# kubernetes-sigs/kube-batch

Hardware: AMD Instinct MI355X
Metric: pod-node scoring evals/sec + binds/sec, 100k tasks x 10k nodes snapshot (higher is better)
Workload: dtype f64+i64

## Files before the change

kube-batch_amd/csrc/kb_commit_sel.hip:

```cpp
#include <string.h>

#include <algorithm>

#include "kb_k9.hpp"
#include "kb_repair.hpp"

#define K9S_PREP0 5u
#define K9S_PREPS 3u
#define K9S_SPIN_LIMIT (1u << 21)

__device__ __forceinline__ uint32_t k9s_ld(const uint32_t *p) { return __hip_atomic_load(p, __ATOMIC_ACQUIRE, __HIP_MEMORY_SCOPE_WORKGROUP); }
__device__ __forceinline__ void k9s_st(uint32_t *p, uint32_t v) { __hip_atomic_store(p, v, __ATOMIC_RELEASE, __HIP_MEMORY_SCOPE_WORKGROUP); }
__device__ __forceinline__ bool k9s_wait(K9Sync &Y, const uint32_t *p, uint32_t need, uint32_t nap = 1u) {
  uint32_t spins = 0;
  for (;;) {
    if (k9s_ld(p) >= need) return true;
    if ((++spins & 31u) == 0u) {
      if (k9s_ld(&Y.stop) | k9s_ld(&Y.err)) return k9s_ld(p) >= need;
      if (spins > K9S_SPIN_LIMIT) { k9s_st(&Y.err, 1u); return false; }
    }
    if (nap == 0u) { } else if (nap == 1u) __builtin_amdgcn_s_sleep(1); else if (nap <= 4u) __builtin_amdgcn_s_sleep(4); else __builtin_amdgcn_s_sleep(16);
  }
}

__global__ void __launch_bounds__(K9_THREADS) k_commit_select(const K9KernArgs ka) {
  KbCommitArgs a = ka.hot;
  {
    const unsigned char __attribute__((address_space(4))) *kp = (const unsigned char __attribute__((address_space(4))) *)__builtin_amdgcn_kernarg_segment_ptr();
    a.dev = (const KbDev *)(kp + offsetof(K9KernArgs, dev));
    a.round = (const KbRound *)(kp + offsetof(K9KernArgs, round));
  }
  extern __shared__ __align__(16) unsigned char k9_smem[];
  if ((blockIdx.x & 7u) != 0u && a.round->lists_ready != nullptr) {
    const uint32_t row = blockIdx.x - 1u - blockIdx.x / 8u;
    if (row < a.n_mrows && !KB_CHAIN_BROKEN(*a.round)) kb_repair_row<K9_THREADS>(*a.dev, *a.round, k9_smem, row, threadIdx.x);
    return;
  }
  if (k9_preamble(a)) return;
  const uint32_t tid = threadIdx.x, lane = tid & 63, wave = tid >> 6;
  const uint32_t S = a.n_mrows, W = a.n_rows;
  const K9Layout lo = k9_layout(W, S, a.L, a.NP, a.R, true);
  unsigned char *k9_base_ = k9_smem;
  K9_LDS_VIEWS(lo)
  (void)shp; (void)S; (void)dk; (void)ckey; (void)cpos;
  K9Sel &X = *reinterpret_cast<K9Sel *>(k9_smem + lo.sel);
  K9Sync &Y = X.sync;
  const unsigned long long t_start = wall_clock64();
#ifdef KB_K9_TRACE
  unsigned long long t_stage[2] = {0ull, 0ull};
  const bool staged = k9_prologue(a, lo, k9_smem, tid, 0u, t_stage);
#else
  const bool staged = k9_prologue(a, lo, k9_smem, tid, 0u);
#endif
  if (!staged) {
    if (tid == 0) k9_publish_skipped(a);
    return;
  }

  uint32_t job_of_my_row = 0u;
  if (tid < W) job_of_my_row = a.dev->t_job[desc[tid].task];
  if (tid < 8) { X.brk[tid] = 0u; X.stm[tid] = 0u; }
  if (tid < 4) { X.stat[tid] = 0u; X.tr[tid] = 0u; }
  if (tid < sizeof(K9Sync) / 4) reinterpret_cast<uint32_t *>(&Y)[tid] = 0u;
  __syncthreads();
  if (tid < W) {
    bool brk = tid == 0;
    if (tid) {
      const KbRowDesc &p = desc[tid - 1], &q = desc[tid];
      const bool plain = (p.flags & 1u) && (p.resmask == 0u || (p.flags & 4u));
      brk = !(plain && !(p.flags & 2u) && q.slot == p.slot && q.flags == p.flags && q.resmask == p.resmask);
    }
    if (brk) atomicOr(&X.brk[tid >> 5], 1u << (tid & 31));
  }
  __syncthreads();
  if (tid < W) {
    uint32_t w = tid >> 5, mword = X.brk[w] & (0xFFFFFFFFu >> (31u - (tid & 31u)));
    while (mword == 0u) { w--; mword = X.brk[w]; }
    const uint32_t p = 32u * w + (31u - (uint32_t)__clz((int)mword));
    if ((tid - p) % K9_SEL_MAXRUN == 0u) atomicOr(&X.stm[tid >> 5], 1u << (tid & 31));
  }
  __syncthreads();
  if (tid < W && ((X.stm[tid >> 5] >> (tid & 31)) & 1u)) {
    uint32_t kidx = (uint32_t)__popc(X.stm[tid >> 5] & ((1u << (tid & 31)) - 1u));
    for (uint32_t w = 0; w < (tid >> 5); w++) kidx += (uint32_t)__popc(X.stm[w]);
    X.runs[kidx] = (uint16_t)tid;
  }
  __syncthreads();
  uint32_t K = 0;
  for (uint32_t w = 0; w < 8; w++) K += (uint32_t)__popc(X.stm[w]);
  {
    uint4 rr = make_uint4(0u, 0u, 0u, 0u);
    uint32_t i0c = 0u;
    uint32_t rlen = 0u;
    if (tid < K) { i0c = X.runs[tid]; rr = rinfo[i0c]; rlen = ((tid + 1u < K) ? (uint32_t)X.runs[tid + 1u] : W) - i0c; }
    __syncthreads();
    if (tid < K) rinfo[tid] = make_uint4(i0c | (rlen << 16), rr.y, rr.z, rr.w);
    __syncthreads();
  }

#ifdef KB_K9_TRACE
  uint32_t tacc[10] = {0, 0, 0, 0, 0, 0, 0, 0, 0, 0};
  const unsigned long long t_tab = wall_clock64();
  tacc[1] = (uint32_t)(t_stage[0] - t_start); tacc[9] = (uint32_t)(t_stage[1] - t_stage[0]); tacc[2] = (uint32_t)(t_tab - t_stage[1]);
  unsigned long long tlast = __builtin_readcyclecounter();
#define K9S_TR(k, t0) do { if (lane == 0) atomicAdd(&X.tr[k], (uint32_t)(__builtin_readcyclecounter() - (t0))); } while (0)
#define K9S_NOW() __builtin_readcyclecounter()
#else
#define K9S_TR(k, t0) do { (void)(t0); } while (0)
#define K9S_NOW() 0ull
#endif
#ifndef KB_K9_NAP_PREP
#define KB_K9_NAP_PREP 1u
#endif
  constexpr uint32_t nap_prep = KB_K9_NAP_PREP, nap_dk = 1u;
#if !defined(KB_K9_PRIO) || KB_K9_PRIO
#define K9S_SETPRIO(p) __builtin_amdgcn_s_setprio(p)
#else
#define K9S_SETPRIO(p) do { } while (0)
#endif
  const unsigned long long lt = (1ull << lane) - 1ull;
  gptrd gi, gr;
  { const KbDev &d = *a.dev; gi = (gptrd)d.idle; gr = (gptrd)d.rel; }
#define K9S_RUN_HEADER_OF(ri_)                                                                                         \
  const uint32_t hx_ = (uint32_t)__builtin_amdgcn_readfirstlane((int)(ri_).x);                                          \
  const uint32_t i0 = hx_ & 0xFFFFu, r = hx_ >> 16, s = (uint32_t)__builtin_amdgcn_readfirstlane((int)(ri_).y);          \
  const uint32_t fl0 = (uint32_t)__builtin_amdgcn_readfirstlane((int)(ri_).z), km0 = (uint32_t)__builtin_amdgcn_readfirstlane((int)(ri_).w); \
  const bool plain0 = (fl0 & 1u) && (km0 == 0u || (fl0 & 4u));                                                         \
  const bool sel_run = !a.backfill && plain0 && r >= 2u && a.whole;             \
  (void)sel_run; (void)i0;
#define K9S_RUN_SHAPE(kk)                                                                                              \
  const K9Shape sh = shapes[s];                                                                                        \
  const double *si = sinit + (size_t)s * RS;                                                                           \
  const double *rres = rowres + ((kk) % K9S_PREPS) * (uint32_t)a.R;    \
  const double *rqv = plain0 ? si : rres + 2;                                             \
  (void)rqv; (void)rres;
#define K9S_RUN_HEADER(kk)                                                                                             \
  const uint4 ri_ = rinfo[(kk)];                                                                                       \
  K9S_RUN_HEADER_OF(ri_)                                                                                               \
  K9S_RUN_SHAPE(kk)

  if (wave == 0) {
    K9S_SETPRIO(3);
    uint32_t nd = 0, n_dirty_rows = 0, n_runs = 0, n_slow = 0, i_end = 0, reason_end = KB_REASON_DONE;
    uint32_t prev_nd0 = 0, prev_pc = 0;
    bool prev_chg = true;
    bool prev_all = false;
    uint4 hd_next = rinfo[0];
    for (uint32_t k = 0; k < K; k++) {
      uint32_t lane_i = tid;
      asm volatile("" : "+v"(lane_i));
      const uint4 hd = hd_next;
      if (k + 1u < K) hd_next = rinfo[k + 1u];
      K9S_RUN_HEADER_OF(hd)
      K9_STAMP(3);
      {
        uint32_t spins = 0;
        bool ok = true;
        for (;;) {
          const uint32_t *wp = (lane_i == 0u) ? (prev_all ? &Y.seq_spec : &Y.seq_cand) : (prev_chg ? &Y.seq_dk[(lane_i - 1u) & 3u] : &Y.seq_early[(lane_i - 1u) & 3u]);
          const uint32_t v = (lane_i < 5u) ? k9s_ld(wp) : 0xFFFFFFFFu;
          if (__ballot(v < k + 1u) == 0ull) break;
          if ((++spins & 31u) == 0u && (k9s_ld(&Y.err) || spins > K9S_SPIN_LIMIT)) { k9s_st(&Y.err, 1u); ok = false; break; }
          __builtin_amdgcn_s_sleep(1);
        }
        if (!ok) { reason_end = KB_REASON_INTERNAL; i_end = i0; break; }
      }
      if (prev_all && lane_i == 0) k9s_st(&Y.seq_cand, k + 1u);
// ... 320 lines not shown
          else if (lane_i == F_PORTS) cur8 |= sh.want;
          else if (lane_i == F_CLS_LEFT) cur8 -= (1ull << 32);
          uint32_t bulk = 1u;
          if (bf_bulk) {
            const uint32_t left1 = (uint32_t)(rl64(cur8, F_CLS_LEFT) >> 32);
            bulk = 1u + min(r - j - 1u, left1);
            if (bulk > 1u) {
              if (lane_i == F_NZC) { double z = u2d(cur8); for (uint32_t t = 1; t < bulk; t++) z += sh.nzc; cur8 = d2u(z); }
              else if (lane_i == F_NZM) { double z = u2d(cur8); for (uint32_t t = 1; t < bulk; t++) z += sh.nzm; cur8 = d2u(z); }
              else if (lane_i == F_CLS_LEFT) cur8 -= ((unsigned long long)(bulk - 1u) << 32);
            }
          }
          if (lane_i < K9_NF) st[lane_i] = cur8;
          if (lane_i < bulk) ldec[i0 + j + lane_i] = (unsigned long long)n | ((unsigned long long)kind << 32);
          j += bulk - 1u;
          n_dirty += bulk - 1u;
          K9_WAVE_FENCE();
          const bool more = j + 1u < r && !kind;
          const uint32_t adjm1 = (!kind && has_map) ? km0 : 0u;
          uint32_t nk = 0u;
          if (more) nk = k9_eval_v(a, sh, k9_load(st), scs, gi, gr, si, adjm1, 1.0, rqv, nb, nmaskbits);
          if (km0 && has_map) {
            if (sc_lane && ((km0 >> sd) & 1u)) k9_sc_sub(kind ? gr : gi, a.NP, sd, n, rqv[sd]);
            sc_dirty = 1;
          }
          if (more) {
            if (lane_i == L) {
              if (is_new) k1 = nk;
              else if (wsel == 0) d0 = nk; else if (wsel == 1) d1 = nk; else if (wsel == 2) d2 = nk; else d3 = nk;
            }
            m = wave_max_u32(max(max(max(d0, d1), max(d2, d3)), (lane_i < pc) ? k1 : 0u));
          }
          n_dirty++;
        }
        if (kind) { j++; reason = KB_REASON_PIPELINED; break; }
      }
      }
      if (sc_dirty) __threadfence();
      const uint32_t i_next = i0 + j;
      uint32_t stop = (reason != KB_REASON_DONE || k + 1u >= K) ? 1u : 0u;
      if (!stop && a.has_aff && !a.backfill && i_next != 0u) {
        const uint32_t fln = (uint32_t)__builtin_amdgcn_readfirstlane((int)hd_next.z);
        if (fln & 2u) { reason = KB_REASON_RENORM; stop = 1u; }
      }
      if (pc) { const uint32_t cp = rl32(cpos, pc - 1u); if (lane_i == 0) cursor[s] = cp + 1u; }
      prev_nd0 = nd; prev_pc = pc; prev_all = pc == ncand;
      K9_WAVE_FENCE();
      prev_chg = chg_any;
      nd += pc; n_dirty_rows += n_dirty; n_runs += 1u; n_slow += plain0 ? 0u : 1u;
      i_end = i_next; reason_end = reason;
      if (lane_i == 0) {
        Y.nd_at[(k + 1u) & 3u] = nd;
        Y.spec_ok[(k + 1u) & 3u] = prev_all ? 1u : 0u;
        if (stop) k9s_st(&Y.stop, 1u);
        k9s_st(&Y.seq_done, k + 1u);
      }
      if (stop) break;
    }
#ifdef KB_K9_TRACE
    tacc[4] = (uint32_t)(wall_clock64() - t_tab);
#endif
    if (lane == 0) {
      if (k9s_ld(&Y.err)) reason_end = KB_REASON_INTERNAL;
      k9s_st(&Y.stop, 1u);
      H.i = i_end; H.nd = nd; H.reason = reason_end; H.n_dirty_rows = n_dirty_rows; H.n_runs = n_runs; H.n_slow = n_slow;
    }
  } else if (wave <= 4u) {
    K9S_SETPRIO(2);
    const uint32_t t = tid - 64u;
    for (uint32_t q = 0; q < K; q++) {
      K9S_RUN_HEADER(q)
      uint32_t *dko = X.dkb[q & 1u];
      uint32_t key = 0u, nd_early = 0u;
      const unsigned long long tw0 = K9S_NOW();
      if (q >= 1u) {
        if (!k9s_wait(Y, &Y.seq_done, q - 1u, nap_dk) || !k9s_wait(Y, &Y.seq_cand, q, nap_dk) || k9s_ld(&Y.stop)) break;
        nd_early = Y.nd_at[(q - 1u) & 3u] + Y.ncand_at[(q - 1u) & 3u];
        if (t < nd_early) {
          const K9St vs = k9_load(slots + (size_t)t * K9_NF);
          const K9Sc scp = k9_sc_preload(sh.active >> 2, gi, gr, a.NP, vs.node);
          key = k9_eval_v(a, sh, vs, scp, gi, gr, si, 0u, 0.0, si, nb, nmaskbits);
          dko[t] = key;
        }
        const uint32_t wmo = wave_max_u32(t < Y.nd_at[(q - 1u) & 3u] ? key : 0u);
        if (lane == 0) Y.mdko[q & 1u][wave - 1u] = wmo;
      }
      if (lane == 0) k9s_st(&Y.seq_early[wave - 1u], q + 1u);
      if (wave == 1u) K9S_TR(3, tw0);
      const unsigned long long tw1 = K9S_NOW();
      if (!k9s_wait(Y, &Y.seq_done, q, nap_dk) || k9s_ld(&Y.stop)) break;
      if (wave == 1u) K9S_TR(2, tw1);
      const uint32_t nd = Y.nd_at[q & 3u];
      if (t < nd && (t >= nd_early || ((Y.chg[(q - 1u) & 1u][t >> 5] >> (t & 31)) & 1u))) {
        const K9St vs = k9_load(slots + (size_t)t * K9_NF);
        const K9Sc scp = k9_sc_preload(sh.active >> 2, gi, gr, a.NP, vs.node);
        key = k9_eval_v(a, sh, vs, scp, gi, gr, si, 0u, 0.0, si, nb, nmaskbits);
      }
      if (t >= nd) key = 0u;
      if (t < K9_MAXSLOTS) dko[t] = key;
      const uint32_t wm = wave_max_u32(key);
      if (lane == 0) { Y.mdk[q & 1u][wave - 1u] = wm; k9s_st(&Y.seq_dk[wave - 1u], q + 1u); }
    }
  } else if (wave < K9S_PREP0 + K9S_PREPS) {
    typedef const unsigned long long __attribute__((address_space(1))) *gptr8;
    typedef const uint32_t __attribute__((address_space(1))) *gptr4;
    gptr8 g8[10];
    gptr8 gports;
    gptr4 gcls, gmaxp, gpodc, gnm;
    {
      const KbDev &d = *a.dev;
      g8[0] = (gptr8)reinterpret_cast<const unsigned long long *>(d.idle); g8[1] = (gptr8)reinterpret_cast<const unsigned long long *>(d.idle + d.NP);
      g8[2] = (gptr8)reinterpret_cast<const unsigned long long *>(d.rel); g8[3] = (gptr8)reinterpret_cast<const unsigned long long *>(d.rel + d.NP);
      g8[4] = (gptr8)reinterpret_cast<const unsigned long long *>(d.inv_acpu); g8[5] = (gptr8)reinterpret_cast<const unsigned long long *>(d.inv_amem);
      g8[6] = (gptr8)reinterpret_cast<const unsigned long long *>(d.acpu); g8[7] = (gptr8)reinterpret_cast<const unsigned long long *>(d.amem);
      g8[8] = (gptr8)reinterpret_cast<const unsigned long long *>(d.nzc); g8[9] = (gptr8)reinterpret_cast<const unsigned long long *>(d.nzm);
      gports = (gptr8)d.ports;
      gcls = (gptr4)d.ncls; gmaxp = (gptr4)reinterpret_cast<const uint32_t *>(d.maxpods); gpodc = (gptr4)reinterpret_cast<const uint32_t *>(d.podcnt); gnm = (gptr4)d.nmask;
    }
    K9Prep &P = X.prep[wave - K9S_PREP0];
    for (uint32_t m = wave - K9S_PREP0; m < K; m += K9S_PREPS) {
      K9S_RUN_HEADER(m)
      const uint32_t r1 = m >= 1u ? (uint32_t)X.runs[m] - (uint32_t)X.runs[m - 1u] : 0u, r2 = m >= 2u ? (uint32_t)X.runs[m - 1u] - (uint32_t)X.runs[m - 2u] : 0u;
      uint32_t want = r + r1 + r2, need = m >= 2u ? m - 2u : 0u;
      if (want > 64u) { want = r + r1; need = m >= 1u ? m - 1u : 0u; }
      const unsigned long long tp0 = K9S_NOW();
      if (!k9s_wait(Y, &Y.seq_done, need, nap_prep) || k9s_ld(&Y.stop)) break;
      K9S_TR(1, tp0);
      uint32_t nf = 0;
      {
        uint32_t e_ = cursor[s];
        while (nf < want) {
          const uint32_t pos_ = e_ + lane;
          const uint32_t kk_ = (pos_ < Lp) ? lists[s * Lp + pos_] : 0u;
          const bool nz_ = kk_ != 0u;
          const uint32_t nn_ = nmaskbits - (kk_ & nmaskbits);
          const bool cl_ = nz_ && !((bitmap[(nz_ ? nn_ : 0u) >> 5] >> (nn_ & 31)) & 1u);
          const unsigned long long zeros_ = __ballot(!nz_);
          const uint32_t fz_ = zeros_ ? (uint32_t)__ffsll((unsigned long long)zeros_) - 1u : 64u;
          const unsigned long long clean_ = __ballot(cl_ && lane < fz_);
          const uint32_t rank_ = (uint32_t)__popcll(clean_ & lt);
          if (((clean_ >> lane) & 1ull) && nf + rank_ < want) { P.ckey[nf + rank_] = kk_; P.cpos[nf + rank_] = pos_; }
          nf = min(want, nf + (uint32_t)__popcll(clean_));
          if (fz_ < 64u || e_ + 64u >= Lp) break;
          e_ += 64u;
        }
        K9_WAVE_FENCE();
      }
      const uint32_t key = (lane < nf) ? P.ckey[lane] : 0u, mypos = (lane < nf) ? P.cpos[lane] : 0u;
      const uint32_t n = nmaskbits - (key & nmaskbits);
      unsigned long long raw[11] = {0, 0, 0, 0, 0, 0, 0, 0, 0, 0, 0};
      uint32_t rcls = 0, rmaxp = 0, rpodc = 0, rnm = 0;
      if (lane < nf) {
#pragma unroll
        for (int f = 0; f < 10; f++) raw[f] = g8[f][n];
        raw[F_PORTS] = gports ? gports[n] : 0ull;
// ... 109 lines not shown
```

kube-batch_amd/csrc/kb_engine.cpp:

```cpp
#include "kb_engine_int.hpp"

thread_local std::string g_create_err;

namespace kbe {

void ensure_window_buffers(kb_engine *e, uint32_t rows) {
  if (rows <= e->win_cap) return;
  if (!e->b_desc.p) e->b_desc.alloc(sizeof(KbRowDesc) * 2 * KB_K5_MAX_WINDOW);
  e->h_rows.resize(rows);
  e->h_slot.resize(rows);
  e->h_decnode.resize(rows);
  e->h_deckind.resize(rows);
  e->win_cap = rows;
}
void ensure_ip_scratch(kb_engine *e, size_t rows) {
  if (!e->hs.has_interpod) return;
  const size_t NP = e->dev.NP;
  if (e->b_ip_scnt.bytes < sizeof(long long) * rows * NP) {
    e->b_ip_scnt.alloc(sizeof(long long) * rows * NP);
    e->b_ip_shist.alloc(sizeof(int32_t) * rows * NP);
  }
  e->dev.ip_scratch_cnt = e->b_ip_scnt.as<long long>();
  e->dev.ip_scratch_hist = e->b_ip_shist.as<int32_t>();
}
// ... 130 lines not shown
        else if (ck[0] == 's') eng->commit_pin = KB_COMMIT_SELECT;
        if (eng->commit_pin >= 0) eng->commit_kernel = eng->commit_pin;
      }
      eng->fast_rounds = !(eng->flags & KB_FLAG_SYNC_ROUNDS);
      const char *cr = getenv("KB_CHAIN_ROUNDS");
      eng->chain_rounds = !(cr && cr[0] == '0');
      const char *pb = getenv("KB_PROBE");
      eng->probe_enabled = !(pb && pb[0] == '0');
      const char *ov = getenv("KB_OVERLAP");
      eng->overlap = !(ov && ov[0] == '0');
      const char *fr = getenv("KB_FUSE_REPAIR");
      eng->fuse_repair = !(fr && fr[0] == '0');
      const char *wf = getenv("KB_DEVICE_WATERFILL");
      eng->device_waterfill = !(wf && wf[0] == '0');
    }
    e = eng.release();
  });
  if (rc == KB_OK) *out = e;
  return rc;
}

void kb_engine_destroy(kb_engine *e) {
  if (!e) return;
  if (getenv("KB_K5_STATS"))
    fprintf(stderr, "[kb K5] rounds on the run kernel %llu, on the selection kernel %llu, last dirty share %.3f\n",
            (unsigned long long)e->rounds_run, (unsigned long long)e->rounds_sel, e->dirty_share);
  if (getenv("KB_K5_STATS") && e->rounds_sel)
    fprintf(stderr, "[kb select] runs of >= 2 rows: all picks clean first placements %llu, committed by shots %llu (shots cut short by a table's end %llu; shots %llu)\n",
            (unsigned long long)e->sel_stat[0], (unsigned long long)e->sel_stat[1], (unsigned long long)e->sel_stat[2], (unsigned long long)e->sel_stat[3]);
  if (getenv("KB_K5_STATS"))
    fprintf(stderr, "[kb K5] rounds %llu, rows %llu, dirty slots %llu, dirty-won rows %llu, runs %llu, runs with a row-specific Resreq %llu (%llu)\n",
            (unsigned long long)e->stats.rounds, (unsigned long long)e->stats.decisions, (unsigned long long)e->k5_slots,
            (unsigned long long)e->stats.row_fallbacks, (unsigned long long)e->k5_walks, (unsigned long long)e->k5_rescans,
            (unsigned long long)e->k5_demand);
  if (getenv("KB_K5_STATS")) fprintf(stderr, "[kb overlap] rounds with candidate lists built beside the predecessor's commit %llu, lists that never arrived %llu; repair launches: %.3f ms from their start to the tag seen\n",
                                     (unsigned long long)e->overlapped_rounds, (unsigned long long)e->overlap_faults, e->tl_repair_tag);
  if (getenv("KB_K5_STATS"))
    fprintf(stderr, "[kb host] ms over the engine's life: reset %.2f, allocate up to its first launch %.2f, speculation breaks (answer -> re-planned launch) %.2f, "
            "closing reductions %.2f, waiting for rounds %.2f, backfill up to its first launch %.2f\n", e->tl_reset, e->tl_begin, e->tl_break, e->tl_finish, e->tl_wait, e->tl_backfill);
  if (getenv("KB_K5_STATS"))
    fprintf(stderr, "[kb host] of the start: order machine %.2f, first probe %.2f, first plan %.2f; of the breaks: probe launch + absorb %.2f, waiting for the probe %.2f, re-plan %.2f\n",
            e->tl_begin_parts[0], e->tl_begin_parts[1], e->tl_begin_parts[2], e->tl_break_parts[0], e->tl_break_parts[1], e->tl_break_parts[2]);
  if (getenv("KB_K5_STATS")) fprintf(stderr, "[kb probe] %llu probes, %llu shapes marked dead by them\n", (unsigned long long)e->probes, (unsigned long long)e->probe_deaths);
  if (getenv("KB_K5_STATS") && e->k5_trace[0] > 0) {
    static const char *ph[10] = {"barrier 1 (wave 0's wait)", "evaluate: candidates (wave 0)", "barrier 2", "rows", "prepare the next run",
                                "rows, of runs with scalar dimensions", "runs with scalar dimensions (count)", "evaluate, of runs with scalar dimensions",
                                "dirty-winner entries (count)", "loop top"};
    static const char *ph_sel[10] = {"wave 0 waits for candidates + dirty keys", "staging: lists, descriptors (10 ns units, not clocks)", "run tables (10 ns units)", "rows: serial loop, tail, publish", "wave 0's loop (10 ns units)",
                                    "selection: entries + first rank", "selection: deep passes", "selection: picks + AddTask", "selection: all picks clean", "shape tables (10 ns units)"};
    const double runs = (double)(e->k5_walks ? e->k5_walks : 1);
    for (int k = 0; k < 10; k++) fprintf(stderr, "[kb K5 trace] %-32s %14.0f clocks  (%.0f per run)\n", e->rounds_sel > e->rounds_run ? ph_sel[k] : ph[k], e->k5_trace[k], e->k5_trace[k] / runs);
    static const char *ph_role[4] = {"prep waves wait for their run's turn (sum of 3)", "prep waves wait for the walk's turn (sum of 3)", "wave 1 waits for the previous run", "wave 1 evaluates + publishes"};
    if (e->rounds_sel > e->rounds_run) for (int k = 10; k < 14; k++) fprintf(stderr, "[kb K5 trace] %-32s %14.0f clocks  (%.0f per run)\n", ph_role[k - 10], e->k5_trace[k], e->k5_trace[k] / runs);
  }
  (void)hipSetDevice(e->device);
  delete e;
}

int kb_get_binds(kb_engine *e, uint32_t *task_node_out) {
  if (!e) return KB_E_INVALID;
  return guarded(e, [&]() {
    if (!e->loaded) throw EngineError(KB_E_STATE, "no session loaded");
    quiesce(e);
    HIP_OK(hipMemcpy(task_node_out, e->b_tbind.p, sizeof(uint32_t) * e->hs.T, hipMemcpyDeviceToHost));
    uint64_t nb = 0;
    for (uint32_t t = 0; t < e->hs.T; t++) nb += task_node_out[t] != KB_NONE;
    e->stats.binds = nb;
  });
}

int kb_get_task_state(kb_engine *e, uint8_t *status_out, uint32_t *node_out) {
  if (!e) return KB_E_INVALID;
  return guarded(e, [&]() {
    if (!e->loaded) throw EngineError(KB_E_STATE, "no session loaded");
    quiesce(e);
    if (status_out) HIP_OK(hipMemcpy(status_out, e->b_tstatus.p, e->hs.T, hipMemcpyDeviceToHost));
    if (node_out) HIP_OK(hipMemcpy(node_out, e->b_tnode.p, sizeof(uint32_t) * e->hs.T, hipMemcpyDeviceToHost));
  });
}

int kb_get_node_state(kb_engine *e, double *idle, double *releasing, int64_t *nz_cpu, int64_t *nz_mem, int32_t *pod_cnt) {
  if (!e) return KB_E_INVALID;
  return guarded(e, [&]() {
    if (!e->loaded) throw EngineError(KB_E_STATE, "no session loaded");
    quiesce(e);
    const uint32_t N = e->hs.N, NP = e->dev.NP;
    const int R = e->hs.R;
    if (idle) HIP_OK(hipMemcpy2D(idle, sizeof(double) * N, e->b_idle.p, sizeof(double) * NP, sizeof(double) * N, R, hipMemcpyDeviceToHost));
    if (releasing) HIP_OK(hipMemcpy2D(releasing, sizeof(double) * N, e->b_rel.p, sizeof(double) * NP, sizeof(double) * N, R, hipMemcpyDeviceToHost));
    if (nz_cpu) HIP_OK(hipMemcpy(nz_cpu, e->b_nzc.p, sizeof(int64_t) * N, hipMemcpyDeviceToHost));
    if (nz_mem) HIP_OK(hipMemcpy(nz_mem, e->b_nzm.p, sizeof(int64_t) * N, hipMemcpyDeviceToHost));
    if (pod_cnt) HIP_OK(hipMemcpy(pod_cnt, e->b_podcnt.p, sizeof(int32_t) * N, hipMemcpyDeviceToHost));
  });
}

int kb_get_shares(kb_engine *e, double *job_share, double *queue_share, double *queue_deserved) {
  if (!e) return KB_E_INVALID;
  return guarded(e, [&]() {
    if (!e->loaded) throw EngineError(KB_E_STATE, "no session loaded");
    const HostSession &hs = e->hs;
    if (job_share) std::memcpy(job_share, hs.job_share.data(), sizeof(double) * hs.J);
    if (queue_share) std::memcpy(queue_share, hs.queue_share.data(), sizeof(double) * hs.Q);
    if (queue_deserved)
      for (uint32_t q = 0; q < hs.Q; q++)
        for (int d = 0; d < hs.R; d++) queue_deserved[(size_t)d * hs.Q + q] = hs.deserved[q].get(d);
  });
// ... 25 lines not shown
```

kube-batch_amd/csrc/kb_k9.hpp:

```cpp
#pragma once
#include <hip/hip_runtime.h>
#include <stddef.h>
#include <stdint.h>
#include <stdlib.h>

#include "kb_device.h"
#include "kb_eval.hpp"
#include "kb_warm.hpp"

#define K9_THREADS 512
#define K9_MAXRUN 64
#define K9_SEL_MAXRUN 32
#define K9_MAXSLOTS 256
#define K9_NF 13
enum { F_IDLE0 = 0, F_IDLE1, F_REL0, F_REL1, F_INVAC, F_INVAM, F_AC, F_AM, F_NZC, F_NZM, F_PORTS, F_CLS_LEFT, F_NODE_NMASK };

struct K9Shape {
  double init0, init1, nzc, nzm;
  unsigned long long conf, want;
  uint32_t cls, active, crow, pad;
};

struct K9Hdr {
  uint32_t i, nd, reason, stop;
  uint32_t ncand, n_dirty_rows, n_runs, n_slow;
  uint32_t cur_s, cur_r, cur_fl, cur_km;
};

struct K9Prep {
  uint32_t ckey[64], cpos[64];
};
struct K9Sync {
  uint32_t seq_done;
  uint32_t seq_cand;
  uint32_t seq_dk[4];
  uint32_t seq_early[4];
  uint32_t seq_spec;
  uint32_t spec_ok[4];
  uint32_t stop, err;
  uint32_t nd_at[4];
  uint32_t ncand_at[4];
  uint32_t mdk[2][4];
  uint32_t mdko[2][4];
  uint32_t chg[2][10];
};
struct K9Sel {
  K9Sync sync;
  K9Prep prep[3];
  uint16_t runs[KB_K5_MAX_ROWS];
  uint32_t brk[8], stm[8];
  struct Cand { uint32_t ckey[64], cpos[64], ckind[64], ck1[64], crnm[64]; } cand[2];
  uint32_t dkb[2][K9_MAXSLOTS];
  uint32_t c_slot[64], c_sorted[64];
  alignas(16) uint32_t c_key[64];
  alignas(16) uint32_t e_eff[64];
  uint32_t e_key[64];
  uint32_t pool[K9_MAXSLOTS + 64];
  uint32_t tr[4];
  uint32_t stat[4];
};

struct K9Layout {
  uint32_t slots, rowres, sinit, shapes, desc, rinfo, dec, hdr, dk, ckey, cpos, cursor, shp, lists, bitmap, sel, total;
  uint32_t Lp, RS;
};
__host__ __device__ inline K9Layout k9_layout(uint32_t n_rows, uint32_t n_shapes, uint32_t L, uint32_t NP, int R, bool sel = false) {
  K9Layout o;
  o.RS = R > 2 ? (uint32_t)(R - 2) : 0u;
  o.Lp = L;
  uint32_t off = 0;
  o.slots = off;  off += (n_rows + K9_MAXRUN) * K9_NF * 8u;
  o.rowres = off; off += 3u * (uint32_t)R * 8u;
  o.sinit = off;  off += n_shapes * o.RS * 8u;
  o.shapes = off; off += n_shapes * (uint32_t)sizeof(K9Shape);
  o.desc = off;   off += n_rows * (uint32_t)sizeof(KbRowDesc);
  off = (off + 15u) & ~15u;
  o.rinfo = off;  off += n_rows * 16u;
  o.dec = off;    off += n_rows * 8u;
  o.hdr = off;    off += (uint32_t)sizeof(K9Hdr);
  o.dk = off;     off += K9_MAXSLOTS * 4u;
  o.ckey = off;   off += K9_MAXRUN * 4u;
  o.cpos = off;   off += K9_MAXRUN * 4u;
  o.cursor = off; off += n_shapes * 4u;
  o.shp = off;    off += n_shapes * 4u;
  o.lists = off;  off += n_shapes * o.Lp * 4u;
  o.bitmap = off; off += (NP / 32u) * 4u;
  off = (off + 15u) & ~15u;
  o.sel = 0;
  if (sel) { o.sel = off; off += (uint32_t)sizeof(K9Sel); }
  o.total = (off + 15u) & ~15u;
  return o;
}

__device__ __forceinline__ uint32_t wave_max_u32(uint32_t v) {
#define K9_UMAX(ctrl, row_mask) v = max(v, (uint32_t)__builtin_amdgcn_update_dpp((int)v, (int)v, (ctrl), (row_mask), 0xf, false))
  K9_UMAX(0xB1, 0xf);
  K9_UMAX(0x4E, 0xf);
// ... 135 lines not shown
  if (a.round->chain_expect != 0u && *a.round->chain != a.round->chain_expect) {
    if (threadIdx.x == 0 && blockIdx.x == 0) k9_publish_skipped(a);
    return true;
  }
  if (blockIdx.x != 0) {
    if ((blockIdx.x & 7u) != 0u) return true;
    const uint32_t h = blockIdx.x / 8u - 1u, lines = a.NP / 16;
    if (h >= KB_WARM_HELPERS) return true;
    const uint32_t l0 = (uint32_t)(((unsigned long long)h * lines) / KB_WARM_HELPERS), l1 = (uint32_t)(((unsigned long long)(h + 1) * lines) / KB_WARM_HELPERS);
    const unsigned long long acc = kb_warm_lines(*a.dev, a.keys, 0, l0, l1, threadIdx.x, K9_THREADS);
    if (acc == 0x123456789abcdefull) a.result[15] = 1;
    return true;
  }
  return false;
}

#define K9_LDS_VIEWS(lo)                                                                                           \
  unsigned long long *slots = reinterpret_cast<unsigned long long *>(k9_base_ + lo.slots); \
  double *rowres = reinterpret_cast<double *>(k9_base_ + lo.rowres); \
  double *sinit = reinterpret_cast<double *>(k9_base_ + lo.sinit); \
  K9Shape *shapes = reinterpret_cast<K9Shape *>(k9_base_ + lo.shapes); \
  KbRowDesc *desc = reinterpret_cast<KbRowDesc *>(k9_base_ + lo.desc); \
  uint4 *rinfo = reinterpret_cast<uint4 *>(k9_base_ + lo.rinfo); \
  unsigned long long *ldec = reinterpret_cast<unsigned long long *>(k9_base_ + lo.dec); \
  K9Hdr &H = *reinterpret_cast<K9Hdr *>(k9_base_ + lo.hdr); \
  uint32_t *dk = reinterpret_cast<uint32_t *>(k9_base_ + lo.dk); \
  uint32_t *ckey = reinterpret_cast<uint32_t *>(k9_base_ + lo.ckey); \
  uint32_t *cpos = reinterpret_cast<uint32_t *>(k9_base_ + lo.cpos); \
  uint32_t *cursor = reinterpret_cast<uint32_t *>(k9_base_ + lo.cursor); \
  uint32_t *shp = reinterpret_cast<uint32_t *>(k9_base_ + lo.shp); \
  uint32_t *lists = reinterpret_cast<uint32_t *>(k9_base_ + lo.lists); \
  uint32_t *bitmap = reinterpret_cast<uint32_t *>(k9_base_ + lo.bitmap); \
  const uint32_t RS = lo.RS, Lp = lo.Lp; \
  const uint32_t nb = a.node_bits, nmaskbits = (1u << nb) - 1u;

template <bool ACQ>
__device__ __forceinline__ bool k9_wait_tags(const KbCommitArgs &a, K9Hdr &H, const uint32_t *tags, const uint32_t tag, const uint32_t n, const uint32_t tid) {
  if (tid < n) {
    bool gone = false;
    uint32_t spins = 0;
    while ((ACQ ? __hip_atomic_load(&tags[tid], __ATOMIC_ACQUIRE, __HIP_MEMORY_SCOPE_AGENT) : __hip_atomic_load(&tags[tid], __ATOMIC_RELAXED, __HIP_MEMORY_SCOPE_AGENT)) != tag) {
      __builtin_amdgcn_s_sleep(2);
      if ((++spins & 15u) == 0u) {
        if (a.round->chain_expect != 0u && __hip_atomic_load(a.round->chain, __ATOMIC_RELAXED, __HIP_MEMORY_SCOPE_AGENT) != a.round->chain_expect) { gone = true; break; }
        if (spins > (1u << 22)) { gone = true; break; }
      }
    }
    if (gone) H.stop = 1u;
  }
  __syncthreads();
  return H.stop == 0u;
}

__device__ __forceinline__ bool k9_prologue(const KbCommitArgs &a, const K9Layout &lo, unsigned char *k9_base_, const uint32_t tid, const uint32_t maxrun,
                                            unsigned long long *stamps = nullptr) {
  const uint32_t S = a.n_mrows, W = a.n_rows;
  K9_LDS_VIEWS(lo)
  (void)slots; (void)rowres; (void)ldec; (void)dk; (void)ckey; (void)cpos; (void)RS;
  const bool fused = a.round->lists_ready != nullptr;
  for (uint32_t w = tid; w < a.NP / 32; w += K9_THREADS) bitmap[w] = 0;
  if (tid == 0) { H.i = 0; H.nd = 0; H.reason = KB_REASON_DONE; H.stop = 0; H.ncand = 0; H.n_dirty_rows = 0; H.n_runs = 0; H.n_slow = 0; H.cur_s = 0; H.cur_r = 0; H.cur_fl = 0; H.cur_km = 0; }
  if (fused) {
    __syncthreads();
    if (!k9_wait_tags<true>(a, H, a.round->ready, a.round->ready_tag, S, tid)) return false;
  }
  constexpr uint32_t UD = 4, UL = 16;
  const uint32_t tot = S * Lp;
  auto stage_lists = [&](uint32_t lbase0) {
    for (uint32_t lbase = lbase0; lbase < tot; lbase += K9_THREADS * UL) {
      unsigned long long lv[UL];
#pragma unroll
      for (uint32_t u = 0; u < UL; u++) {
        const unsigned long long *kp = &a.keys[min(lbase + u * K9_THREADS + tid, tot - 1u)];
        lv[u] = fused ? __hip_atomic_load(kp, __ATOMIC_RELAXED, __HIP_MEMORY_SCOPE_AGENT) : *kp;
      }
#pragma unroll
      for (uint32_t u = 0; u < UL; u++) {
        const uint32_t idx = lbase + u * K9_THREADS + tid;
        const unsigned long long k64 = lv[u];
        if (idx < tot) lists[idx] = k64 ? (((KB_KEY_SCORE(k64) + 1u) << nb) | (nmaskbits - KB_KEY_NODE(k64))) : 0u;
      }
    }
  };
  {
    const unsigned long long *dsrc = reinterpret_cast<const unsigned long long *>(a.desc);
    unsigned long long *ddst = reinterpret_cast<unsigned long long *>(desc);
    const uint32_t dwords = W * (uint32_t)(sizeof(KbRowDesc) / 8);
    static_assert(KB_K5_MAX_ROWS * (sizeof(KbRowDesc) / 8) <= K9_THREADS * UD, "the descriptors are staged in one batch");
    unsigned long long dv[UD], lv[UL] = {};
#pragma unroll
    for (uint32_t u = 0; u < UD; u++) dv[u] = dsrc[min(u * K9_THREADS + tid, dwords - 1u)];
    if (!fused && tot) {
#pragma unroll
      for (uint32_t u = 0; u < UL; u++) lv[u] = a.keys[min(u * K9_THREADS + tid, tot - 1u)];
    }
#pragma unroll
    for (uint32_t u = 0; u < UD; u++) { const uint32_t w = u * K9_THREADS + tid; if (w < dwords) ddst[w] = dv[u]; }
    if (!fused) {
#pragma unroll
      for (uint32_t u = 0; u < UL; u++) {
        const uint32_t idx = u * K9_THREADS + tid;
        const unsigned long long k64 = lv[u];
        if (idx < tot) lists[idx] = k64 ? (((KB_KEY_SCORE(k64) + 1u) << nb) | (nmaskbits - KB_KEY_NODE(k64))) : 0u;
      }
      stage_lists(K9_THREADS * UL);
    }
  }
  for (uint32_t s = tid; s < S; s += K9_THREADS) cursor[s] = 0;
  __syncthreads();
  if (stamps) stamps[0] = wall_clock64();
  for (uint32_t i = tid; i < W; i += K9_THREADS) shp[desc[i].slot] = i;
  __syncthreads();
  for (uint32_t s = tid; s < S; s += K9_THREADS) {
    const KbRowDesc &k = desc[shp[s]];
    K9Shape sh;
    sh.init0 = k.init0; sh.init1 = k.init1; sh.nzc = (double)k.nzc; sh.nzm = (double)k.nzm;
    sh.conf = a.has_ports ? a.dev->t_conf[k.task] : 0ull;
    sh.want = a.has_ports ? a.dev->t_want[k.task] : 0ull;
    sh.cls = k.cls; sh.active = k.active; sh.crow = k.crow; sh.pad = 0;
    shapes[s] = sh;
  }
  if (RS) {
    const KbDev &d = *a.dev;
    for (uint32_t idx = tid; idx < S * RS; idx += K9_THREADS) {
      const uint32_t s = idx / RS, dd = idx % RS;
      sinit[idx] = d.t_init[(size_t)(dd + 2) * d.T + desc[shp[s]].task];
    }
  }
  __syncthreads();
  if (stamps) stamps[1] = wall_clock64();

  for (uint32_t i = tid; i < W; i += K9_THREADS) {
    const KbRowDesc &k = desc[i];
    const uint32_t sl = k.slot, fl = k.flags, km = k.resmask;
    const bool plain = (fl & 1u) && (km == 0u || (fl & 4u));
    uint32_t r = 1;
    if (plain && !(fl & 2u))
      while (r < maxrun && i + r < W && desc[i + r].slot == sl && desc[i + r].flags == fl && desc[i + r].resmask == km) r++;
    rinfo[i] = make_uint4(r, sl, fl, km);
  }
  if (fused) {
    if (!k9_wait_tags<false>(a, H, a.round->lists_ready, a.round->lists_tag, S, tid)) return false;
    stage_lists(0u);
  }
  __syncthreads();
  return true;
}

__device__ __forceinline__ void k9_epilogue(const KbCommitArgs &a, const K9Layout &lo, unsigned char *k9_base_, const uint32_t tid, const unsigned long long t_start,
                                            const uint32_t w6, const uint32_t w7, const bool job_known = false, const uint32_t job_of_my_row = 0u) {
  K9_LDS_VIEWS(lo)
  (void)rowres; (void)sinit; (void)shapes; (void)rinfo; (void)dk; (void)ckey; (void)cpos; (void)cursor; (void)shp; (void)lists; (void)bitmap; (void)RS; (void)Lp; (void)nb; (void)nmaskbits;
  const uint32_t n_done = H.i, nd = H.nd;
  const unsigned long long *hdr = reinterpret_cast<const unsigned long long *>(a.result);
  unsigned long long *mh = slots + (size_t)(a.n_rows + K9_MAXRUN - 2u) * K9_NF;
  static_assert(2u * K9_NF >= KB_OUT_HDR, "the header's LDS copy lives in two slots");
  if (a.host_out)
    for (uint32_t i = tid; i < n_done; i += K9_THREADS) a.host_out[KB_OUT_HDR + i] = ldec[i];
  unsigned long long hpre = 0ull;
  if (a.host_out && tid < KB_OUT_HDR) hpre = __hip_atomic_load(const_cast<unsigned long long *>(&hdr[tid]), __ATOMIC_RELAXED, __HIP_MEMORY_SCOPE_AGENT);
  uint32_t my_job = job_of_my_row;
  if (!job_known && tid < n_done) my_job = a.dev->t_job[desc[tid].task];
  {
    const KbDev &d = *a.dev;
    for (uint32_t slot = tid; slot < nd; slot += K9_THREADS) {
      const unsigned long long *sl = slots + (size_t)slot * K9_NF;
      const uint32_t n = (uint32_t)sl[F_NODE_NMASK];
      d.idle[n] = u2d(sl[F_IDLE0]);
      d.idle[(size_t)d.NP + n] = u2d(sl[F_IDLE1]);
      d.rel[n] = u2d(sl[F_REL0]);
      d.rel[(size_t)d.NP + n] = u2d(sl[F_REL1]);
      d.nzc[n] = (long long)u2d(sl[F_NZC]);
      d.nzm[n] = (long long)u2d(sl[F_NZM]);
      d.podcnt[n] = d.maxpods[n] - (int)(uint32_t)(sl[F_CLS_LEFT] >> 32);
      if (a.has_ports) d.ports[n] = sl[F_PORTS];
    }
  }
  {
    const KbDev &d = *a.dev;
    const KbRound &r = *a.round;
    for (uint32_t i = tid; i < n_done; i += K9_THREADS) {
      const unsigned long long rec = ldec[i];
      a.dec[i] = rec;
      const uint32_t n = (uint32_t)rec, kind = (uint32_t)(rec >> 32);
      if (n == KB_NONE_U32) continue;
      const KbRowDesc &k = desc[i];
      const uint32_t t = k.task;
      d.t_status[t] = kind ? KB_TASK_PIPELINED : KB_TASK_ALLOCATED;
      d.t_node[t] = n;
      d.t_counted[t] = 1;
      if (!kind) d.j_allocated[i == tid ? my_job : d.t_job[t]] = 1;
      if (d.t_ip_cls_inc) {
        for (uint32_t w = 0; w < d.ip_Wp; w++) {
          unsigned long long cm = d.t_ip_cls_inc[(size_t)t * d.ip_Wp + w];
          while (cm) {
            const uint32_t pcl = 64u * w + (uint32_t)__ffsll((unsigned long long)cm) - 1u;
            cm &= cm - 1ull;
// ... 91 lines not shown
```

Before: 21.22 billion.

## Defer list staging past run-table setup and skip unneeded final key passes

Under a new default-on flag, the commit-select kernel stops waiting for the fused candidate lists inside the prologue and stages them only after the run table is built. This lets the wait on the repair blocks overlap with the run setup work. The key-evaluation waves now prefetch the next run header and shape, and wait on seq_done, seq_cand, stop and err together with a single ballot instead of separate spin loops. A new need_final flag lets them skip the final re-evaluation pass when the walk changed nothing, which saves evaluation work but adds a new synchronisation contract that must stay correct. Trace-only segment counters and a host readout are also added.

Result: no change. 21.41 billion (median of 3 runs) (+0.9%).

```diff
diff --git a/kube-batch_amd/csrc/kb_commit_sel.hip b/kube-batch_amd/csrc/kb_commit_sel.hip
--- a/kube-batch_amd/csrc/kb_commit_sel.hip
+++ b/kube-batch_amd/csrc/kb_commit_sel.hip
@@ -21,6 +21,35 @@
     }
     if (nap == 0u) { } else if (nap == 1u) __builtin_amdgcn_s_sleep(1); else if (nap <= 4u) __builtin_amdgcn_s_sleep(4); else __builtin_amdgcn_s_sleep(16);
   }
+}
+
+#ifndef KB_K9_DK_LEAN
+#define KB_K9_DK_LEAN 1
+#endif
+__device__ __forceinline__ bool k9s_wait_run(K9Sync &Y, const uint32_t lane, const uint32_t need_done, const uint32_t need_cand) {
+  const uint32_t *wp = lane == 0u ? &Y.seq_done : (lane == 1u ? &Y.seq_cand : (lane == 2u ? &Y.stop : &Y.err));
+  const uint32_t need = lane == 0u ? need_done : (lane == 1u ? need_cand : 0u);
+  uint32_t spins = 0;
+  for (;;) {
+    const uint32_t v = lane < 4u ? k9s_ld(wp) : 0u;
+    const unsigned long long b = __ballot(lane < 2u ? v < need : (lane < 4u && v != 0u));
+    if (b == 0ull) return true;
+    if (b & 0xCull) return false;
+    if (++spins > K9S_SPIN_LIMIT) { if (lane == 0u) k9s_st(&Y.err, 1u); return false; }
+    __builtin_amdgcn_s_sleep(1);
+  }
+}
+
+#ifdef KB_K9_TRACE
+__device__ unsigned long long k9s_trace_acc[8];
+#endif
+extern "C" void kb_sel_trace_words(unsigned long long *out, int n) {
+  for (int i = 0; i < n; i++) out[i] = 0ull;
+#ifdef KB_K9_TRACE
+  unsigned long long w[8];
+  if (hipMemcpyFromSymbol(w, HIP_SYMBOL(k9s_trace_acc), sizeof(w)) == hipSuccess)
+    for (int i = 0; i < n && i < 8; i++) out[i] = w[i];
+#endif
 }
 
 __global__ void __launch_bounds__(K9_THREADS) k_commit_select(const K9KernArgs ka) {
@@ -48,9 +77,9 @@
   const unsigned long long t_start = wall_clock64();
 #ifdef KB_K9_TRACE
   unsigned long long t_stage[2] = {0ull, 0ull};
-  const bool staged = k9_prologue(a, lo, k9_smem, tid, 0u, t_stage);
+  const bool staged = k9_prologue(a, lo, k9_smem, tid, 0u, t_stage, KB_K9_DK_LEAN != 0);
 #else
-  const bool staged = k9_prologue(a, lo, k9_smem, tid, 0u);
+  const bool staged = k9_prologue(a, lo, k9_smem, tid, 0u, nullptr, KB_K9_DK_LEAN != 0);
 #endif
   if (!staged) {
     if (tid == 0) k9_publish_skipped(a);
@@ -61,7 +90,8 @@
   if (tid < W) job_of_my_row = a.dev->t_job[desc[tid].task];
   if (tid < 8) { X.brk[tid] = 0u; X.stm[tid] = 0u; }
   if (tid < 4) { X.stat[tid] = 0u; X.tr[tid] = 0u; }
-  if (tid < sizeof(K9Sync) / 4) reinterpret_cast<uint32_t *>(&Y)[tid] = 0u;
+  static_assert(sizeof(K9Sync) / 4 <= K9_THREADS, "one thread per word");
+  if (tid < sizeof(K9Sync) / 4) reinterpret_cast<uint32_t *>(&Y)[tid] = (tid == offsetof(K9Sync, need_final) / 4) ? 1u : 0u;
   __syncthreads();
   if (tid < W) {
     bool brk = tid == 0;
@@ -97,6 +127,12 @@
     if (tid < K) rinfo[tid] = make_uint4(i0c | (rlen << 16), rr.y, rr.z, rr.w);
     __syncthreads();
   }
+#if KB_K9_DK_LEAN
+  if (a.round->lists_ready != nullptr && !k9_prologue_lists(a, lo, k9_smem, tid)) {
+    if (tid == 0) k9_publish_skipped(a);
+    return;
+  }
+#endif
 
 #ifdef KB_K9_TRACE
   uint32_t tacc[10] = {0, 0, 0, 0, 0, 0, 0, 0, 0, 0};
@@ -105,14 +141,22 @@
   unsigned long long tlast = __builtin_readcyclecounter();
 #define K9S_TR(k, t0) do { if (lane == 0) atomicAdd(&X.tr[k], (uint32_t)(__builtin_readcyclecounter() - (t0))); } while (0)
 #define K9S_NOW() __builtin_readcyclecounter()
+  uint32_t wseg[8] = {0, 0, 0, 0, 0, 0, 0, 0};
+#define K9S_SEG(k, t0) do { const unsigned long long n_ = __builtin_readcyclecounter(); wseg[k] += (uint32_t)(n_ - (t0)); (t0) = n_; } while (0)
+#define K9S_CNT(k) do { wseg[k] += 1u; } while (0)
+#define K9S_PIN(v) asm volatile("" :: "v"(v))
 #else
 #define K9S_TR(k, t0) do { (void)(t0); } while (0)
 #define K9S_NOW() 0ull
+#define K9S_SEG(k, t0) do { (void)(t0); } while (0)
+#define K9S_CNT(k) do { } while (0)
+#define K9S_PIN(v) do { } while (0)
 #endif
 #ifndef KB_K9_NAP_PREP
 #define KB_K9_NAP_PREP 1u
 #endif
   constexpr uint32_t nap_prep = KB_K9_NAP_PREP, nap_dk = 1u;
+  (void)nap_dk;
 #if !defined(KB_K9_PRIO) || KB_K9_PRIO
 #define K9S_SETPRIO(p) __builtin_amdgcn_s_setprio(p)
 #else
@@ -539,6 +583,7 @@
       if (lane_i == 0) {
         Y.nd_at[(k + 1u) & 3u] = nd;
         Y.spec_ok[(k + 1u) & 3u] = prev_all ? 1u : 0u;
+        Y.need_final[(k + 1u) & 3u] = chg_any ? 1u : 0u;
         if (stop) k9s_st(&Y.stop, 1u);
         k9s_st(&Y.seq_done, k + 1u);
       }
@@ -555,28 +600,89 @@
   } else if (wave <= 4u) {
     K9S_SETPRIO(2);
     const uint32_t t = tid - 64u;
+#if KB_K9_DK_LEAN
+    uint4 hd_next = rinfo[0];
+    K9Shape sh_next = shapes[hd_next.y];
     for (uint32_t q = 0; q < K; q++) {
-      K9S_RUN_HEADER(q)
+      unsigned long long ts = K9S_NOW();
+      const uint4 hd = hd_next;
+      const K9Shape sh = sh_next;
+      if (q + 1u < K) hd_next = rinfo[q + 1u];
+      K9S_RUN_HEADER_OF(hd)
+      const double *si = sinit + (size_t)s * RS;
       uint32_t *dko = X.dkb[q & 1u];
       uint32_t key = 0u, nd_early = 0u;
+      K9S_PIN(sh.pad);
+      K9S_SEG(0, ts);
       const unsigned long long tw0 = K9S_NOW();
       if (q >= 1u) {
-        if (!k9s_wait(Y, &Y.seq_done, q - 1u, nap_dk) || !k9s_wait(Y, &Y.seq_cand, q, nap_dk) || k9s_ld(&Y.stop)) break;
-        nd_early = Y.nd_at[(q - 1u) & 3u] + Y.ncand_at[(q - 1u) & 3u];
+        if (!k9s_wait_run(Y, lane, q - 1u, q)) break;
+        const uint32_t nd_prev = Y.nd_at[(q - 1u) & 3u], nc_prev = Y.ncand_at[(q - 1u) & 3u];
+        nd_early = nd_prev + nc_prev;
+        K9S_PIN(nd_early);
+        K9S_SEG(1, ts);
         if (t < nd_early) {
           const K9St vs = k9_load(slots + (size_t)t * K9_NF);
           const K9Sc scp = k9_sc_preload(sh.active >> 2, gi, gr, a.NP, vs.node);
           key = k9_eval_v(a, sh, vs, scp, gi, gr, si, 0u, 0.0, si, nb, nmaskbits);
           dko[t] = key;
         }
+        const uint32_t wmo = wave_max_u32(t < nd_prev ? key : 0u);
+        if (lane == 0) Y.mdko[q & 1u][wave - 1u] = wmo;
+      }
+      if (lane == 0) k9s_st(&Y.seq_early[wave - 1u], q + 1u);
+      if (wave == 1u) K9S_TR(3, tw0);
+      K9S_SEG(2, ts);
+      if (q + 1u < K) sh_next = shapes[hd_next.y];
+      const unsigned long long tw1 = K9S_NOW();
+      if (!k9s_wait_run(Y, lane, q, 0u)) break;
+      const uint32_t nd = Y.nd_at[q & 3u];
+      const uint32_t nfin = (uint32_t)__builtin_amdgcn_readfirstlane((int)Y.need_final[q & 3u]);
+      if (wave == 1u) K9S_TR(2, tw1);
+      K9S_SEG(3, ts);
+      K9S_CNT(7);
+      if (nfin == 0u) { K9S_CNT(6); continue; }
+      if (t < nd && (t >= nd_early || ((Y.chg[(q - 1u) & 1u][t >> 5] >> (t & 31)) & 1u))) {
+        const K9St vs = k9_load(slots + (size_t)t * K9_NF);
+        const K9Sc scp = k9_sc_preload(sh.active >> 2, gi, gr, a.NP, vs.node);
+        key = k9_eval_v(a, sh, vs, scp, gi, gr, si, 0u, 0.0, si, nb, nmaskbits);
+      }
+      if (t >= nd) key = 0u;
+      if (t < K9_MAXSLOTS) dko[t] = key;
+      const uint32_t wm = wave_max_u32(key);
+      if (lane == 0) { Y.mdk[q & 1u][wave - 1u] = wm; k9s_st(&Y.seq_dk[wave - 1u], q + 1u); }
+      K9S_SEG(4, ts); K9S_CNT(5);
+    }
+#else
+    for (uint32_t q = 0; q < K; q++) {
+      unsigned long long ts = K9S_NOW();
+      K9S_RUN_HEADER(q)
+      uint32_t *dko = X.dkb[q & 1u];
+      uint32_t key = 0u, nd_early = 0u;
+      K9S_PIN(sh.pad);
+      K9S_SEG(0, ts);
+      const unsigned long long tw0 = K9S_NOW();
+      if (q >= 1u) {
+        if (!k9s_wait(Y, &Y.seq_done, q - 1u, nap_dk) || !k9s_wait(Y, &Y.seq_cand, q, nap_dk) || k9s_ld(&Y.stop)) break;
+        nd_early = Y.nd_at[(q - 1u) & 3u] + Y.ncand_at[(q - 1u) & 3u];
+        K9S_PIN(nd_early);
+        K9S_SEG(1, ts);
+        if (t < nd_early) {
+          const K9St vs = k9_load(slots + (size_t)t * K9_NF);
+          const K9Sc scp = k9_sc_preload(sh.active >> 2, gi, gr, a.NP, vs.node);
+          key = k9_eval_v(a, sh, vs, scp, gi, gr, si, 0u, 0.0, si, nb, nmaskbits);
+          dko[t] = key;
+        }
         const uint32_t wmo = wave_max_u32(t < Y.nd_at[(q - 1u) & 3u] ? key : 0u);
         if (lane == 0) Y.mdko[q & 1u][wave - 1u] = wmo;
       }
       if (lane == 0) k9s_st(&Y.seq_early[wave - 1u], q + 1u);
       if (wave == 1u) K9S_TR(3, tw0);
+      K9S_SEG(2, ts);
       const unsigned long long tw1 = K9S_NOW();
       if (!k9s_wait(Y, &Y.seq_done, q, nap_dk) || k9s_ld(&Y.stop)) break;
       if (wave == 1u) K9S_TR(2, tw1);
+      K9S_SEG(3, ts);
       const uint32_t nd = Y.nd_at[q & 3u];
       if (t < nd && (t >= nd_early || ((Y.chg[(q - 1u) & 1u][t >> 5] >> (t & 31)) & 1u))) {
         const K9St vs = k9_load(slots + (size_t)t * K9_NF);
@@ -587,7 +693,13 @@
       if (t < K9_MAXSLOTS) dko[t] = key;
       const uint32_t wm = wave_max_u32(key);
       if (lane == 0) { Y.mdk[q & 1u][wave - 1u] = wm; k9s_st(&Y.seq_dk[wave - 1u], q + 1u); }
+      K9S_SEG(4, ts); K9S_CNT(5); K9S_CNT(7);
     }
+#endif
+#ifdef KB_K9_TRACE
+    if (tid == 64u)
+      for (uint32_t i = 0; i < 8u; i++) atomicAdd(&k9s_trace_acc[i], (unsigned long long)wseg[i]);
+#endif
   } else if (wave < K9S_PREP0 + K9S_PREPS) {
     typedef const unsigned long long __attribute__((address_space(1))) *gptr8;
     typedef const uint32_t __attribute__((address_space(1))) *gptr4;
diff --git a/kube-batch_amd/csrc/kb_engine.cpp b/kube-batch_amd/csrc/kb_engine.cpp
--- a/kube-batch_amd/csrc/kb_engine.cpp
+++ b/kube-batch_amd/csrc/kb_engine.cpp
@@ -206,6 +206,16 @@
     for (int k = 0; k < 10; k++) fprintf(stderr, "[kb K5 trace] %-32s %14.0f clocks  (%.0f per run)\n", e->rounds_sel > e->rounds_run ? ph_sel[k] : ph[k], e->k5_trace[k], e->k5_trace[k] / runs);
     static const char *ph_role[4] = {"prep waves wait for their run's turn (sum of 3)", "prep waves wait for the walk's turn (sum of 3)", "wave 1 waits for the previous run", "wave 1 evaluates + publishes"};
     if (e->rounds_sel > e->rounds_run) for (int k = 10; k < 14; k++) fprintf(stderr, "[kb K5 trace] %-32s %14.0f clocks  (%.0f per run)\n", ph_role[k - 10], e->k5_trace[k], e->k5_trace[k] / runs);
+    if (e->rounds_sel > e->rounds_run) {
+      extern void kb_sel_trace_words(unsigned long long *out, int n) __attribute__((weak));
+      unsigned long long w[8] = {0, 0, 0, 0, 0, 0, 0, 0};
+      (void)hipSetDevice(e->device);
+      if (kb_sel_trace_words) kb_sel_trace_words(w, 8);
+      static const char *seg[5] = {"wave 1: run header", "wave 1: waits in front of the early evaluation", "wave 1: early evaluation up to seq_early", "wave 1: wait for seq_done q", "wave 1: final pass up to seq_dk"};
+      const double wr = (double)(w[7] ? w[7] : 1ull);
+      for (int k = 0; k < 5; k++) fprintf(stderr, "[kb K5 trace] %-48s %14llu clocks  (%.0f per run of %llu)\n", seg[k], w[k], (double)w[k] / wr, w[7]);
+      fprintf(stderr, "[kb K5 trace] wave 1: final passes run %llu, skipped %llu; loop per run %.0f clocks\n", w[5], w[6], (double)(w[0] + w[1] + w[2] + w[3] + w[4]) / wr);
+    }
   }
   (void)hipSetDevice(e->device);
   delete e;
diff --git a/kube-batch_amd/csrc/kb_k9.hpp b/kube-batch_amd/csrc/kb_k9.hpp
--- a/kube-batch_amd/csrc/kb_k9.hpp
+++ b/kube-batch_amd/csrc/kb_k9.hpp
@@ -43,6 +43,7 @@
   uint32_t mdk[2][4];
   uint32_t mdko[2][4];
   uint32_t chg[2][10];
+  uint32_t need_final[4];
 };
 struct K9Sel {
   K9Sync sync;
@@ -284,8 +285,28 @@
   return H.stop == 0u;
 }
 
+#define K9_STAGE_UL 16u
+__device__ __forceinline__ void k9_stage_lists(const KbCommitArgs &a, uint32_t *lists, const uint32_t tot, const uint32_t nb, const uint32_t nmaskbits, const bool fused,
+                                               const uint32_t lbase0, const uint32_t tid) {
+  constexpr uint32_t UL = K9_STAGE_UL;
+  for (uint32_t lbase = lbase0; lbase < tot; lbase += K9_THREADS * UL) {
+    unsigned long long lv[UL];
+#pragma unroll
+    for (uint32_t u = 0; u < UL; u++) {
+      const unsigned long long *kp = &a.keys[min(lbase + u * K9_THREADS + tid, tot - 1u)];
+      lv[u] = fused ? __hip_atomic_load(kp, __ATOMIC_RELAXED, __HIP_MEMORY_SCOPE_AGENT) : *kp;
+    }
+#pragma unroll
+    for (uint32_t u = 0; u < UL; u++) {
+      const uint32_t idx = lbase + u * K9_THREADS + tid;
+      const unsigned long long k64 = lv[u];
+      if (idx < tot) lists[idx] = k64 ? (((KB_KEY_SCORE(k64) + 1u) << nb) | (nmaskbits - KB_KEY_NODE(k64))) : 0u;
+    }
+  }
+}
+
 __device__ __forceinline__ bool k9_prologue(const KbCommitArgs &a, const K9Layout &lo, unsigned char *k9_base_, const uint32_t tid, const uint32_t maxrun,
-                                            unsigned long long *stamps = nullptr) {
+                                            unsigned long long *stamps = nullptr, const bool lists_later = false) {
   const uint32_t S = a.n_mrows, W = a.n_rows;
   K9_LDS_VIEWS(lo)
   (void)slots; (void)rowres; (void)ldec; (void)dk; (void)ckey; (void)cpos; (void)RS;
@@ -296,24 +317,9 @@
     __syncthreads();
     if (!k9_wait_tags<true>(a, H, a.round->ready, a.round->ready_tag, S, tid)) return false;
   }
-  constexpr uint32_t UD = 4, UL = 16;
+  constexpr uint32_t UD = 4, UL = K9_STAGE_UL;
   const uint32_t tot = S * Lp;
-  auto stage_lists = [&](uint32_t lbase0) {
-    for (uint32_t lbase = lbase0; lbase < tot; lbase += K9_THREADS * UL) {
-      unsigned long long lv[UL];
-#pragma unroll
-      for (uint32_t u = 0; u < UL; u++) {
-        const unsigned long long *kp = &a.keys[min(lbase + u * K9_THREADS + tid, tot - 1u)];
-        lv[u] = fused ? __hip_atomic_load(kp, __ATOMIC_RELAXED, __HIP_MEMORY_SCOPE_AGENT) : *kp;
-      }
-#pragma unroll
-      for (uint32_t u = 0; u < UL; u++) {
-        const uint32_t idx = lbase + u * K9_THREADS + tid;
-        const unsigned long long k64 = lv[u];
-        if (idx < tot) lists[idx] = k64 ? (((KB_KEY_SCORE(k64) + 1u) << nb) | (nmaskbits - KB_KEY_NODE(k64))) : 0u;
-      }
-    }
-  };
+  auto stage_lists = [&](uint32_t lbase0) { k9_stage_lists(a, lists, tot, nb, nmaskbits, fused, lbase0, tid); };
   {
     const unsigned long long *dsrc = reinterpret_cast<const unsigned long long *>(a.desc);
     unsigned long long *ddst = reinterpret_cast<unsigned long long *>(desc);
@@ -371,10 +377,19 @@
       while (r < maxrun && i + r < W && desc[i + r].slot == sl && desc[i + r].flags == fl && desc[i + r].resmask == km) r++;
     rinfo[i] = make_uint4(r, sl, fl, km);
   }
-  if (fused) {
+  if (fused && !lists_later) {
     if (!k9_wait_tags<false>(a, H, a.round->lists_ready, a.round->lists_tag, S, tid)) return false;
     stage_lists(0u);
   }
+  __syncthreads();
+  return true;
+}
+__device__ __forceinline__ bool k9_prologue_lists(const KbCommitArgs &a, const K9Layout &lo, unsigned char *k9_base_, const uint32_t tid) {
+  const uint32_t S = a.n_mrows;
+  K9_LDS_VIEWS(lo)
+  (void)slots; (void)rowres; (void)sinit; (void)shapes; (void)desc; (void)rinfo; (void)ldec; (void)dk; (void)ckey; (void)cpos; (void)cursor; (void)shp; (void)bitmap; (void)RS;
+  if (!k9_wait_tags<false>(a, H, a.round->lists_ready, a.round->lists_tag, S, tid)) return false;
+  k9_stage_lists(a, lists, S * Lp, nb, nmaskbits, true, 0u, tid);
   __syncthreads();
   return true;
 }
```
